# secondlaw-ai/skyrim

Hardware: AMD Instinct MI355X
Metric: 6-h forecast steps/sec on 721x1440 state, 1/2/4/8 MI355X; per-channel max rel-err vs ref (higher is better)
Workload: dtype f16; 1 GPU; Pangu 6-h autoregressive rollout, 721x1440x69 state (13 levels x 5 vars + 4 surface), random-init weights (64 M params), state resident in HBM, 1 ensemble membe; parallelism=single GPU, members=1, finite=True, rounding=compensated, term_plan=0x66f

## Files before the change

### skyrim_amd/csrc/attention.hip

```cpp
#include <cstdlib>
#include "gemm_dma.h"
#include "launchers.h"

namespace skp {

__device__ __forceinline__ int attn_key(int f, int row) {
    return f < 8 ? 32 * (f >> 1) + 8 * (row >> 2) + 4 * (f & 1) + (row & 3) : 128 + row;
}

__device__ __forceinline__ void attn_softmax_pv(f32x4 (&s)[9], const uint4 (&vf)[2][5], f32x4 (&o)[2], f32x4& osum) {
    typedef f16 T;
    const float LOG2E = 1.4426950408889634f;
    float mx = s[0][0];
#pragma unroll
    for (int f = 0; f < 9; ++f)
#pragma unroll
        for (int r = 0; r < 4; ++r) mx = fmaxf(mx, s[f][r]);
    mx = fmaxf(mx, __shfl_xor(mx, 16));
    mx = fmaxf(mx, __shfl_xor(mx, 32));
    const float mxl = mx * LOG2E;
#pragma unroll
    for (int f = 0; f < 9; ++f)
#pragma unroll
        for (int r = 0; r < 4; ++r) s[f][r] = __builtin_amdgcn_exp2f(__builtin_fmaf(s[f][r], LOG2E, -mxl));
    o[0] = f32x4{0.f, 0.f, 0.f, 0.f}; o[1] = f32x4{0.f, 0.f, 0.f, 0.f}; osum = f32x4{0.f, 0.f, 0.f, 0.f};
    const uint4 ones = make_uint4(0x3C003C00u, 0x3C003C00u, 0x3C003C00u, 0x3C003C00u);
#pragma unroll
    for (int kb = 0; kb < 5; ++kb) {
        float pv[8];
#pragma unroll
        for (int r = 0; r < 4; ++r) {
            pv[r] = s[2 * kb][r];
            pv[4 + r] = (kb < 4) ? s[(2 * kb + 1) % 9][r] : 0.f;
        }
        uint4 pf[1];
        split8<T, 1>(pv, pf);
#pragma unroll
        for (int df = 0; df < 2; ++df) o[df] = OpT<T>::mfma(as_v8<T>(vf[df][kb]), as_v8<T>(pf[0]), o[df]);
        osum = OpT<T>::mfma(as_v8<T>(ones), as_v8<T>(pf[0]), osum);
    }
}

constexpr int BT_ROW = 28, BT_COPY = 144 * BT_ROW + 120;

template <class TO, int NPL_O>
__global__ void __launch_bounds__(256) __attribute__((amdgpu_waves_per_eu(3, 3))) earth_attention2_kernel(const f16* __restrict__ q, const f16* __restrict__ k,
                                                              const f16* __restrict__ vt, const f16* __restrict__ bias_cmp, TO* __restrict__ out,
                                                              long long out_plane, int ld_out, int nW, int heads) {
    typedef f16 T;
    __shared__ __attribute__((aligned(16))) f16 tabs[4 * BT_COPY];
    const int lane = threadIdx.x & 63, wave = threadIdx.x >> 6;
    const int th = blockIdx.x;
    const int head = th % heads, type = th / heads;
    const int l15 = lane & 15, g = lane >> 4;
    {
        const f16* src = bias_cmp + (long long)th * 3456;
        for (int i = threadIdx.x; i < 3456; i += 256) {
            const int r = i / 24, e = i - 24 * r;
            const f16 v = src[i];
            if (e < 23) {
#pragma unroll
                for (int c = 0; c < 4; ++c) tabs[c * BT_COPY + r * BT_ROW + e + c] = v;
            }
        }
    }
    int koff[9];
#pragma unroll
    for (int f = 0; f < 9; ++f) {
        const int k0 = f < 8 ? 32 * (f >> 1) + 8 * g + 4 * (f & 1) : 128 + 4 * g;
        const int zk = k0 / 72, hk = (k0 / 12) % 6, wk0 = k0 % 12;
        koff[f] = 2 * ((2 * zk * 36 + 6 * hk) * BT_ROW + wk0);
    }
    __syncthreads();
    const char* tb = reinterpret_cast<const char*>(tabs);

    for (int wi = wave; wi < nW; wi += 4) {
        const int win = type * nW + wi;
        const long long base = (long long)win * heads + head;
        const T* qp = q + base * (WIN_TOKENS * HEAD_DIM) + l15 * HEAD_DIM + g * 8;
        const T* kp = k + base * (WIN_TOKENS * HEAD_DIM) + g * 8;
        const T* vp = vt + base * (WIN_TOKENS * HEAD_DIM) + (8 * (l15 >> 2) + (l15 & 3)) * WIN_TOKENS;

        uint4 kf[9];
#pragma unroll
        for (int f = 0; f < 9; ++f) kf[f] = *reinterpret_cast<const uint4*>(kp + attn_key(f, l15) * HEAD_DIM);
        uint4 vf[2][5];
#pragma unroll
        for (int df = 0; df < 2; ++df)
#pragma unroll
            for (int kb = 0; kb < 5; ++kb) {
                const T* s = vp + df * 4 * WIN_TOKENS;
                if (kb < 4) vf[df][kb] = *reinterpret_cast<const uint4*>(s + kb * 32 + g * 8);
                else { const uint2 lo = *reinterpret_cast<const uint2*>(s + 128 + g * 4); vf[df][kb] = make_uint4(lo.x, lo.y, 0, 0); }
            }
        uint4 qn = *reinterpret_cast<const uint4*>(qp);
#pragma unroll 1
        for (int qf = 0; qf < 9; ++qf) {
            const uint4 qv = qn;
            if (qf < 8) qn = *reinterpret_cast<const uint4*>(qp + (qf + 1) * 16 * HEAD_DIM);
            const int qi = 16 * qf + l15;
            const int zq = qi >= 72 ? 1 : 0, hq = (qi - 72 * zq) / 12, wq = qi - 72 * zq - 12 * hq;
            const int c = (wq + 1) & 3;
            const char* bq = tb + 2 * (c * BT_COPY + (zq * 36 + hq) * BT_ROW + (11 - wq) + c);
            uint2 bias[9];
#pragma unroll
            for (int f = 0; f < 9; ++f) bias[f] = *reinterpret_cast<const uint2*>(bq + koff[f]);

            f32x4 s[9];
#pragma unroll
            for (int f = 0; f < 9; ++f) {
                typedef f16 h4 __attribute__((ext_vector_type(4)));
                const h4 b = __builtin_bit_cast(h4, bias[f]);
                s[f] = OpT<T>::mfma(as_v8<T>(kf[f]), as_v8<T>(qv), f32x4{(float)b[0], (float)b[1], (float)b[2], (float)b[3]});
            }
            f32x4 o[2], osum;
            attn_softmax_pv(s, vf, o, osum);
            const float inv = __builtin_amdgcn_rcpf(osum[0]);
            TO* orow = out + blk_off((long long)win * WIN_TOKENS + qf * 16 + l15, head * HEAD_DIM, ld_out) + g * 8;
            const float y[8] = {o[0][0] * inv, o[0][1] * inv, o[0][2] * inv, o[0][3] * inv, o[1][0] * inv, o[1][1] * inv, o[1][2] * inv, o[1][3] * inv};
            store8_planes<TO, NPL_O>(orow, out_plane, y);
        }
    }
}


template <int C_, int PL_>
struct QaShape {
    static constexpr int C = C_, PL = PL_, KS = C / 32, NWAVES = 8, THREADS = 64 * NWAVES;
    static constexpr int BLK_KIB = KS * 2 * PL;
    static constexpr int W_BYTES = 3 * BLK_KIB * 1024;
    static constexpr int TAB_BYTES = (4 * BT_COPY * 2 + 1023) / 1024 * 1024;
    static constexpr int RING_BYTES = 6 * 1024;
    static constexpr int SMEM = W_BYTES + TAB_BYTES + 1024 + NWAVES * RING_BYTES;
    static_assert(SMEM <= 160 * 1024, "LDS");
};

struct QkvAttnArgs {
    const f16* xs;
    const int* widx;
    const f16* wf;
    const float* bias;
    const f16* bias_cmp;
    const f16* zrow;
    f16* out; long long out_plane;
    int nW, heads, types;
    float scale;
};

template <class S, int NPL_O>
__global__ void __launch_bounds__(S::THREADS) __attribute__((amdgpu_waves_per_eu(2, 2)))
qkv_attention_kernel(const QkvAttnArgs a) {
    typedef f16 T;
    constexpr int C = S::C, KS = S::KS, PL = S::PL;
    extern __shared__ __attribute__((aligned(16))) char smem[];
    char* wl = smem;
    f16* tabs = reinterpret_cast<f16*>(smem + S::W_BYTES);
    float* qb = reinterpret_cast<float*>(smem + S::W_BYTES + S::TAB_BYTES);
    const int tid = threadIdx.x, lane = tid & 63, l15 = lane & 15, g = lane >> 4;
    const int wave = __builtin_amdgcn_readfirstlane(tid >> 6);
    const int xcd = blockIdx.x & 7, slot = blockIdx.x >> 3;
    const int head = slot % a.heads, type = xcd + 8 * (slot / a.heads);
    if (type >= a.types) return;
    const int th = type * a.heads + head;
    {
        const unsigned lds_base = (unsigned)(size_t)smem;
#pragma unroll
        for (int which = 0; which < 3; ++which) {
            const f16* src = a.wf + ((long long)(which * a.heads + head) * S::BLK_KIB << 9) + lane * 8;
            for (int p = wave; p < S::BLK_KIB; p += S::NWAVES) glds16(src + (p << 9), lds_base + (unsigned)((which * S::BLK_KIB + p) << 10));
        }
        const f16* src = a.bias_cmp + (long long)th * 3456;
        constexpr int NT = (3456 + S::THREADS - 1) / S::THREADS;
        f16 tv[NT];
#pragma unroll
        for (int j = 0; j < NT; ++j) { const int i = tid + j * S::THREADS; tv[j] = src[i < 3456 ? i : 0]; }
#pragma unroll
        for (int j = 0; j < NT; ++j) {
            const int i = tid + j * S::THREADS;
            const int r = i / 24, e = i - 24 * r;
            if (i < 3456 && e < 23) {
#pragma unroll
                for (int c = 0; c < 4; ++c) tabs[c * BT_COPY + r * BT_ROW + e + c] = tv[j];
            }
        }
        if (tid < 96) qb[tid] = a.bias[(tid >> 5) * C + head * HEAD_DIM + (tid & 31)];
    }
    int koff[9];
#pragma unroll
    for (int f = 0; f < 9; ++f) {
        const int k0 = f < 8 ? 32 * (f >> 1) + 8 * g + 4 * (f & 1) : 128 + 4 * g;
        const int zk = k0 / 72, hk = (k0 / 12) % 6, wk0 = k0 % 12;
        koff[f] = 2 * ((2 * zk * 36 + 6 * hk) * BT_ROW + wk0);
    }
    int srcn[9];
    auto load_src = [&](int wi_) {
        const int w_ = type * a.nW + wi_;
#pragma unroll
        for (int f = 0; f < 9; ++f) srcn[f] = a.widx[w_ * WIN_TOKENS + attn_key(f, l15)];
    };
    load_src(wave < a.nW ? wave : 0);
    asm volatile("s_waitcnt vmcnt(0)" ::: "memory");
    __syncthreads();
    const char* tb = reinterpret_cast<const char*>(tabs);
    const char* wrd = wl + lane * 16;
    const unsigned ring_base = (unsigned)(size_t)smem + (unsigned)(S::W_BYTES + S::TAB_BYTES + 1024 + wave * S::RING_BYTES);
    const char* ring_rd = smem + S::W_BYTES + S::TAB_BYTES + 1024 + wave * S::RING_BYTES + lane * 16;

    for (int wi = wave; wi < a.nW; wi += S::NWAVES) {
        const int win = type * a.nW + wi;
        int src[9];
#pragma unroll
        for (int f = 0; f < 9; ++f) src[f] = srcn[f];
        typedef unsigned u32x9 __attribute__((ext_vector_type(9)));
        u32x9 qx, qy, qz, qw;
        uint4 kf[9];
        uint2 vh[9][2];
        const T* xp[3];
        int xstep[3];
        auto point = [&](int tg_) {
#pragma unroll
            for (int i = 0; i < 3; ++i) {
                const int r = src[3 * tg_ + i];
                xp[i] = r >= 0 ? a.xs + blk_off(r, g * 8, C) : a.zrow;
                xstep[i] = r >= 0 ? 512 : 0;
            }
        };
        auto fetch = [&](int ks) {
#pragma unroll
            for (int i = 0; i < 3; ++i) glds16(xp[i] + ks * xstep[i], ring_base + (unsigned)(((ks & 1) * 3 + i) << 10));
        };
        point(0);
        fetch(0);
        fetch(1);
#pragma unroll
        for (int tg = 0; tg < 3; ++tg) {
            f32x4 qa[3][2], ka[3][2], va[3][2];
#pragma unroll
            for (int i = 0; i < 3; ++i)
#pragma unroll
                for (int n = 0; n < 2; ++n) { qa[i][n] = f32x4{0.f, 0.f, 0.f, 0.f}; ka[i][n] = f32x4{0.f, 0.f, 0.f, 0.f}; va[i][n] = f32x4{0.f, 0.f, 0.f, 0.f}; }
#pragma unroll 1
            for (int ks = 0; ks < KS; ++ks) {
                if (ks + 1 < KS) asm volatile("s_waitcnt vmcnt(3)" ::: "memory");
                else asm volatile("s_waitcnt vmcnt(0)" ::: "memory");
                uint4 xf[3];
#pragma unroll
                for (int i = 0; i < 3; ++i) xf[i] = *reinterpret_cast<const uint4*>(ring_rd + (((ks & 1) * 3 + i) << 10));
                if (ks + 2 < KS) {
                    asm volatile("s_waitcnt lgkmcnt(0)" ::: "memory");
                    fetch(ks + 2);
                }
#pragma unroll
                for (int which = 0; which < 3; ++which)
#pragma unroll
                    for (int n = 0; n < 2; ++n)
#pragma unroll
                        for (int p = PL - 1; p >= 0; --p) {
                            const uint4 w = *reinterpret_cast<const uint4*>(wrd + ((((which * KS + ks) * 2 + n) * PL + p) << 10));
#pragma unroll
                            for (int i = 0; i < 3; ++i) {
                                if (which == 0) qa[i][n] = OpT<T>::mfma(as_v8<T>(w), as_v8<T>(xf[i]), qa[i][n]);
                                else if (which == 1) ka[i][n] = OpT<T>::mfma(as_v8<T>(w), as_v8<T>(xf[i]), ka[i][n]);
                                else va[i][n] = OpT<T>::mfma(as_v8<T>(xf[i]), as_v8<T>(w), va[i][n]);
                            }
                        }
            }
            if (tg < 2) {
                point(tg + 1);
                fetch(0);
                fetch(1);
            }
            float bq[8], bk[8], bv[2];
#pragma unroll
            for (int i = 0; i < 8; ++i) { bq[i] = qb[8 * g + i]; bk[i] = qb[32 + 8 * g + i]; }
#pragma unroll
            for (int df = 0; df < 2; ++df) bv[df] = qb[64 + 8 * (l15 >> 2) + 4 * df + (l15 & 3)];
#pragma unroll
            for (int i = 0; i < 3; ++i) {
                const int f = 3 * tg + i;
                float v[8];
                uint4 o[1];
#pragma unroll
                for (int r = 0; r < 4; ++r) { v[r] = (qa[i][0][r] + bq[r]) * a.scale; v[4 + r] = (qa[i][1][r] + bq[4 + r]) * a.scale; }
                split8<T, 1>(v, o);
                asm volatile("" : "+v"(o[0].x), "+v"(o[0].y), "+v"(o[0].z), "+v"(o[0].w));
                qx[f] = o[0].x; qy[f] = o[0].y; qz[f] = o[0].z; qw[f] = o[0].w;
#pragma unroll
                for (int r = 0; r < 4; ++r) { v[r] = ka[i][0][r] + bk[r]; v[4 + r] = ka[i][1][r] + bk[4 + r]; }
                split8<T, 1>(v, o);
                kf[f] = o[0];
#pragma unroll
                for (int df = 0; df < 2; ++df) {
                    const float u[4] = {va[i][df][0] + bv[df], va[i][df][1] + bv[df], va[i][df][2] + bv[df], va[i][df][3] + bv[df]};
                    uint2 h[1];
                    split4<T, 1>(u, h);
                    vh[f][df] = h[0];
                }
                asm volatile("" : "+v"(kf[f].x), "+v"(kf[f].y), "+v"(kf[f].z), "+v"(kf[f].w), "+v"(vh[f][0].x), "+v"(vh[f][0].y), "+v"(vh[f][1].x), "+v"(vh[f][1].y));
            }
        }
        uint4 vf[2][5];
#pragma unroll
        for (int df = 0; df < 2; ++df) {
#pragma unroll
            for (int kb = 0; kb < 4; ++kb) vf[df][kb] = make_uint4(vh[2 * kb][df].x, vh[2 * kb][df].y, vh[2 * kb + 1][df].x, vh[2 * kb + 1][df].y);
            vf[df][4] = make_uint4(vh[8][df].x, vh[8][df].y, 0, 0);
        }
        if (wi + S::NWAVES < a.nW) load_src(wi + S::NWAVES);
#pragma unroll 1
        for (int qf = 0; qf < 9; ++qf) {
            const uint4 qc = make_uint4(qx[qf], qy[qf], qz[qf], qw[qf]);
            const int qi = attn_key(qf, l15);
            const int zq = qi >= 72 ? 1 : 0, hq = (qi - 72 * zq) / 12, wq = qi - 72 * zq - 12 * hq;
            const int c = (wq + 1) & 3;
            const char* bqp = tb + 2 * (c * BT_COPY + (zq * 36 + hq) * BT_ROW + (11 - wq) + c);
            f32x4 s[9];
#pragma unroll
            for (int f = 0; f < 9; ++f) {
                typedef f16 h4 __attribute__((ext_vector_type(4)));
                const h4 b = __builtin_bit_cast(h4, *reinterpret_cast<const uint2*>(bqp + koff[f]));
                s[f] = OpT<T>::mfma(as_v8<T>(kf[f]), as_v8<T>(qc), f32x4{(float)b[0], (float)b[1], (float)b[2], (float)b[3]});
            }
            f32x4 o[2], osum;
            attn_softmax_pv(s, vf, o, osum);
            const float inv = __builtin_amdgcn_rcpf(osum[0]);
            T* orow = a.out + blk_off((long long)win * WIN_TOKENS + qi, head * HEAD_DIM, C) + g * 8;
            const float y[8] = {o[0][0] * inv, o[0][1] * inv, o[0][2] * inv, o[0][3] * inv, o[1][0] * inv, o[1][1] * inv, o[1][2] * inv, o[1][3] * inv};
            store8_planes<T, NPL_O>(orow, a.out_plane, y);
        }
    }
}

template <class S>
static hipError_t launch_qa(const QkvAttnArgs& a, int types, int out_planes, hipStream_t stream) {
    if (out_planes == 1) {
        auto kern = qkv_attention_kernel<S, 1>;
        hipError_t e = hipFuncSetAttribute(reinterpret_cast<const void*>(kern), hipFuncAttributeMaxDynamicSharedMemorySize, S::SMEM);
        if (e != hipSuccess) return e;
        hipLaunchKernelGGL(kern, dim3((unsigned)(8 * ((types + 7) / 8) * a.heads)), dim3(S::THREADS), S::SMEM, stream, a);
    } else {
        auto kern = qkv_attention_kernel<S, 2>;
        hipError_t e = hipFuncSetAttribute(reinterpret_cast<const void*>(kern), hipFuncAttributeMaxDynamicSharedMemorySize, S::SMEM);
        if (e != hipSuccess) return e;
        hipLaunchKernelGGL(kern, dim3((unsigned)(8 * ((types + 7) / 8) * a.heads)), dim3(S::THREADS), S::SMEM, stream, a);
    }
    return hipGetLastError();
}

hipError_t op_qkv_attention(const Geom& g, const BlockW<f16>& b, const int* widx, int res, const f16* Xs, const Work<PrecF16x3>& wk, hipStream_t s, int out_planes) {
    if (!b.bias_cmp || !(b.qkvh || b.qkvf)) return hipErrorInvalidValue;
    const int heads = res == 0 ? 6 : 12;
    QkvAttnArgs a{Xs, widx, b.qkvh ? b.qkvh : b.qkvf, b.qkv_b, b.bias_cmp, wk.zrow, wk.ao, wk.ao_plane, g.nW[res], heads, g.types[res], 0.17677669529663687f};
    if (b.qkvh) return res == 0 ? launch_qa<QaShape<192, 1>>(a, g.types[res], out_planes, s) : launch_qa<QaShape<384, 1>>(a, g.types[res], out_planes, s);
    if (res != 0) return hipErrorNotSupported;
    return launch_qa<QaShape<192, 2>>(a, g.types[res], out_planes, s);
}

template <class P>
hipError_t launch_attention(const AttnArgs<P>& a, hipStream_t stream) {
    constexpr int NPL_O = (P::NA > P::NW ? P::NA : P::NW);
    const int types = a.n_win / a.nW;
    if (a.out_planes == 1)
        hipLaunchKernelGGL((earth_attention2_kernel<typename P::T, 1>), dim3((unsigned)(types * a.heads)), dim3(256), 0, stream,
                           a.q, a.k, a.vt, a.bias_cmp, a.out, a.out_plane, a.ld_out, a.nW, a.heads);
    else
        hipLaunchKernelGGL((earth_attention2_kernel<typename P::T, NPL_O>), dim3((unsigned)(types * a.heads)), dim3(256), 0, stream,
                           a.q, a.k, a.vt, a.bias_cmp, a.out, a.out_plane, a.ld_out, a.nW, a.heads);
    return hipGetLastError();
}

template hipError_t launch_attention<PrecBF16x3>(const AttnArgs<PrecBF16x3>&, hipStream_t);
template hipError_t launch_attention<PrecF16x3>(const AttnArgs<PrecF16x3>&, hipStream_t);

}
```

### skyrim_amd/csrc/common.h

```cpp
#pragma once
#include <hip/hip_runtime.h>
#include <stdint.h>

namespace skp {

typedef _Float16 f16;
typedef __bf16 bf16;
typedef float f32x4 __attribute__((ext_vector_type(4)));
typedef f16 f16x8 __attribute__((ext_vector_type(8)));
typedef bf16 bf16x8 __attribute__((ext_vector_type(8)));

template <class T> struct OpT;
template <> struct OpT<f16> {
    typedef f16x8 v8;
    static __device__ __forceinline__ f32x4 mfma(v8 a, v8 b, f32x4 c) {
        return __builtin_amdgcn_mfma_f32_16x16x32_f16(a, b, c, 0, 0, 0);
    }
};
template <> struct OpT<bf16> {
    typedef bf16x8 v8;
    static __device__ __forceinline__ f32x4 mfma(v8 a, v8 b, f32x4 c) {
        return __builtin_amdgcn_mfma_f32_16x16x32_bf16(a, b, c, 0, 0, 0);
    }
};

template <class T>
__device__ __forceinline__ typename OpT<T>::v8 as_v8(const uint4& u) {
    return __builtin_bit_cast(typename OpT<T>::v8, u);
}

struct PrecBF16x3 { typedef bf16 T; static constexpr int NA = 2, NW = 2; };
struct PrecF16x3  { typedef f16 T;  static constexpr int NA = 2, NW = 2; };
struct PrecF16x2W { typedef f16 T;  static constexpr int NA = 1, NW = 2; };

__device__ __forceinline__ void load8(const float* p, float (&v)[8]) {
    const float4 a = *reinterpret_cast<const float4*>(p), b = *reinterpret_cast<const float4*>(p + 4);
    v[0] = a.x; v[1] = a.y; v[2] = a.z; v[3] = a.w; v[4] = b.x; v[5] = b.y; v[6] = b.z; v[7] = b.w;
}

template <class T, int NP>
__device__ __forceinline__ void split8(const float (&v)[8], uint4 (&out)[NP]) {
    typename OpT<T>::v8 h;
#pragma unroll
    for (int i = 0; i < 8; ++i) h[i] = (T)v[i];
    if constexpr (NP == 2) asm volatile("" : "+v"(h));
    out[0] = __builtin_bit_cast(uint4, h);
    if constexpr (NP == 2) {
        typename OpT<T>::v8 l;
#pragma unroll
        for (int i = 0; i < 8; ++i) l[i] = (T)(v[i] - (float)h[i]);
        out[1] = __builtin_bit_cast(uint4, l);
    }
}

template <class T, int NP>
__device__ __forceinline__ void split4(const float (&v)[4], uint2 (&out)[NP]) {
    typedef T t4 __attribute__((ext_vector_type(4)));
    t4 h;
#pragma unroll
    for (int i = 0; i < 4; ++i) h[i] = (T)v[i];
    if constexpr (NP == 2) asm volatile("" : "+v"(h));
    out[0] = __builtin_bit_cast(uint2, h);
    if constexpr (NP == 2) {
        t4 l;
#pragma unroll
        for (int i = 0; i < 4; ++i) l[i] = (T)(v[i] - (float)h[i]);
        out[1] = __builtin_bit_cast(uint2, l);
    }
}

template <class S>
__device__ __forceinline__ void store4(S* p, const float (&v)[4]) {
    if constexpr (sizeof(S) == 4) {
        *reinterpret_cast<float4*>(p) = make_float4(v[0], v[1], v[2], v[3]);
    } else {
        uint2 o[1];
        split4<S, 1>(v, o);
        *reinterpret_cast<uint2*>(p) = o[0];
    }
}

__device__ __host__ __forceinline__ long long blk_off(long long row, int col, int K) {
    return (((row >> 4) * (K >> 5) + (col >> 5)) << 9) + ((row & 15) << 5) + (col & 31);
}

template <class T, int NP>
__device__ __forceinline__ void store4_planes(T* p, long long plane, const float (&v)[4]) {
    uint2 o[NP];
    split4<T, NP>(v, o);
    *reinterpret_cast<uint2*>(p) = o[0];
    if constexpr (NP == 2) *reinterpret_cast<uint2*>(p + plane) = o[1];
}

template <class T, int NP>
__device__ __forceinline__ void store8_planes(T* p, long long plane, const float (&v)[8]) {
    uint4 o[NP];
    split8<T, NP>(v, o);
    *reinterpret_cast<uint4*>(p) = o[0];
    if constexpr (NP == 2) *reinterpret_cast<uint4*>(p + plane) = o[1];
}

__device__ __host__ __forceinline__ int perm8_col(int rho) {
    const int r = rho & 31;
    return (rho & ~31) + 8 * ((r >> 2) & 3) + 4 * (r >> 4) + (r & 3);
}

template <int BK>
__device__ __forceinline__ int lds_off(int row, int slot) {
    if constexpr (BK == 64) return row * 128 + ((slot ^ (row & 7)) << 4);
    else                    return row * 64 + ((slot ^ ((row >> 1) & 3)) << 4);
}

typedef float f32x2 __attribute__((ext_vector_type(2)));
__device__ __forceinline__ f32x2 gelu_erf2(f32x2 x) {
    f32x2 a;
    a.x = __builtin_amdgcn_fmed3f(__builtin_fabsf(x.x), 0.f, 5.9396970f);
    a.y = __builtin_amdgcn_fmed3f(__builtin_fabsf(x.y), 0.f, 5.9396970f);
    f32x2 p = __builtin_elementwise_fma(a, (f32x2)(-6.177511978e-07f), (f32x2)(1.091520153e-05f));
    p = __builtin_elementwise_fma(a, p, (f32x2)(-4.273382365e-05f));
    p = __builtin_elementwise_fma(a, p, (f32x2)(-4.982745158e-04f));
    p = __builtin_elementwise_fma(a, p, (f32x2)(7.545167115e-03f));
    p = __builtin_elementwise_fma(a, p, (f32x2)(-5.282834917e-02f));
    p = __builtin_elementwise_fma(a, p, (f32x2)(-4.591012597e-01f));
    p = __builtin_elementwise_fma(a, p, (f32x2)(-1.151117682e+00f));
    p = p * a;
    f32x2 t;
    t.x = 1.0f - __builtin_amdgcn_exp2f(p.x);
    t.y = 1.0f - __builtin_amdgcn_exp2f(p.y);
    t.x = __builtin_copysignf(t.x, x.x);
    t.y = __builtin_copysignf(t.y, x.y);
    return ((f32x2)(0.5f) * x) * ((f32x2)(1.0f) + t);
}
__device__ __forceinline__ float gelu_erf(float x) { return gelu_erf2((f32x2){x, x}).x; }
__device__ __forceinline__ f32x2 gelu_erf2e(f32x2 x) {
    f32x2 a;
    a.x = __builtin_amdgcn_fmed3f(__builtin_fabsf(x.x), 0.f, 5.9396970f);
    a.y = __builtin_amdgcn_fmed3f(__builtin_fabsf(x.y), 0.f, 5.9396970f);
    const f32x2 a2 = a * a;
    const f32x2 q01 = __builtin_elementwise_fma(a, (f32x2)(-4.591012597e-01f), (f32x2)(-1.151117682e+00f));
    const f32x2 q23 = __builtin_elementwise_fma(a, (f32x2)(7.545167115e-03f), (f32x2)(-5.282834917e-02f));
    const f32x2 q45 = __builtin_elementwise_fma(a, (f32x2)(-4.273382365e-05f), (f32x2)(-4.982745158e-04f));
    const f32x2 q67 = __builtin_elementwise_fma(a, (f32x2)(-6.177511978e-07f), (f32x2)(1.091520153e-05f));
    const f32x2 a4 = a2 * a2;
    const f32x2 q03 = __builtin_elementwise_fma(a2, q23, q01);
    const f32x2 q47 = __builtin_elementwise_fma(a2, q67, q45);
    f32x2 p = __builtin_elementwise_fma(a4, q47, q03);
    p = p * a;
    f32x2 t;
    t.x = 1.0f - __builtin_amdgcn_exp2f(p.x);
    t.y = 1.0f - __builtin_amdgcn_exp2f(p.y);
    t.x = __builtin_copysignf(t.x, x.x);
    t.y = __builtin_copysignf(t.y, x.y);
    return ((f32x2)(0.5f) * x) * ((f32x2)(1.0f) + t);
}
__device__ __forceinline__ void gelu_erf8(const f32x4& lo, const f32x4& hi, float (&v)[8]) {
    const f32x2 r0 = gelu_erf2((f32x2){lo[0], lo[1]}), r1 = gelu_erf2((f32x2){lo[2], lo[3]});
    const f32x2 r2 = gelu_erf2((f32x2){hi[0], hi[1]}), r3 = gelu_erf2((f32x2){hi[2], hi[3]});
    v[0] = r0.x; v[1] = r0.y; v[2] = r1.x; v[3] = r1.y; v[4] = r2.x; v[5] = r2.y; v[6] = r3.x; v[7] = r3.y;
}

constexpr int WIN_TOKENS = 144;
constexpr int HEAD_DIM = 32;

}
```

Before: 75.76 steps/s.

## Precompute attention lane geometry in LDS and prefetch next bias tile

The fused QKV-attention kernel now precomputes per-lane query geometry (bias-table offset and output offset) into a small LDS table instead of recomputing integer divisions per query fragment. It prefetches the next fragment's relative-position bias into registers while the current one runs softmax. The softmax row max uses permlane16/32 swap instructions with fmed3-based max in place of shuffles. The first K-step is peeled so accumulators are zero-initialised through the MFMA operand instead of explicit zeroing. The cost is more register pressure and a reshuffled LDS layout.

```diff
diff --git a/skyrim_amd/csrc/attention.hip b/skyrim_amd/csrc/attention.hip
--- a/skyrim_amd/csrc/attention.hip
+++ b/skyrim_amd/csrc/attention.hip
@@ -1,23 +1,27 @@
 #include <cstdlib>
+#include <type_traits>
 #include "gemm_dma.h"
 #include "launchers.h"
 
 namespace skp {
 
-__device__ __forceinline__ int attn_key(int f, int row) {
-    return f < 8 ? 32 * (f >> 1) + 8 * (row >> 2) + 4 * (f & 1) + (row & 3) : 128 + row;
-}
-
+template <bool SWAP>
 __device__ __forceinline__ void attn_softmax_pv(f32x4 (&s)[9], const uint4 (&vf)[2][5], f32x4 (&o)[2], f32x4& osum) {
     typedef f16 T;
     const float LOG2E = 1.4426950408889634f;
-    float mx = s[0][0];
+    float mx = SWAP ? max_raw(s[0][0], s[0][1]) : s[0][0];
 #pragma unroll
     for (int f = 0; f < 9; ++f)
 #pragma unroll
-        for (int r = 0; r < 4; ++r) mx = fmaxf(mx, s[f][r]);
-    mx = fmaxf(mx, __shfl_xor(mx, 16));
-    mx = fmaxf(mx, __shfl_xor(mx, 32));
+        for (int r = 0; r < 4; ++r)
+            if (!SWAP || 4 * f + r >= 2) mx = fmaxf(mx, s[f][r]);
+    if constexpr (SWAP) {
+        mx = xlane_max_swap<16>(mx);
+        mx = xlane_max_swap<32>(mx);
+    } else {
+        mx = fmaxf(mx, __shfl_xor(mx, 16));
+        mx = fmaxf(mx, __shfl_xor(mx, 32));
+    }
     const float mxl = mx * LOG2E;
 #pragma unroll
     for (int f = 0; f < 9; ++f)
@@ -41,7 +45,6 @@
     }
 }
 
-constexpr int BT_ROW = 28, BT_COPY = 144 * BT_ROW + 120;
 
 template <class TO, int NPL_O>
 __global__ void __launch_bounds__(256) __attribute__((amdgpu_waves_per_eu(3, 3))) earth_attention2_kernel(const f16* __restrict__ q, const f16* __restrict__ k,
@@ -114,7 +117,7 @@
                 s[f] = OpT<T>::mfma(as_v8<T>(kf[f]), as_v8<T>(qv), f32x4{(float)b[0], (float)b[1], (float)b[2], (float)b[3]});
             }
             f32x4 o[2], osum;
-            attn_softmax_pv(s, vf, o, osum);
+            attn_softmax_pv<false>(s, vf, o, osum);
             const float inv = __builtin_amdgcn_rcpf(osum[0]);
             TO* orow = out + blk_off((long long)win * WIN_TOKENS + qf * 16 + l15, head * HEAD_DIM, ld_out) + g * 8;
             const float y[8] = {o[0][0] * inv, o[0][1] * inv, o[0][2] * inv, o[0][3] * inv, o[1][0] * inv, o[1][1] * inv, o[1][2] * inv, o[1][3] * inv};
@@ -130,9 +133,11 @@
     static constexpr int BLK_KIB = KS * 2 * PL;
     static constexpr int W_BYTES = 3 * BLK_KIB * 1024;
     static constexpr int TAB_BYTES = (4 * BT_COPY * 2 + 1023) / 1024 * 1024;
+    static constexpr int GEO_BYTES = 9 * 64 * 8;
     static constexpr int RING_BYTES = 6 * 1024;
-    static constexpr int SMEM = W_BYTES + TAB_BYTES + 1024 + NWAVES * RING_BYTES;
-    static_assert(SMEM <= 160 * 1024, "LDS");
+    static constexpr int GEO_OFF = W_BYTES + TAB_BYTES, QB_OFF = GEO_OFF + GEO_BYTES, RING_OFF = GEO_OFF + 5 * 1024;
+    static constexpr int SMEM = RING_OFF + NWAVES * RING_BYTES;
+    static_assert(GEO_BYTES <= 4608 && GEO_OFF % 8 == 0 && QB_OFF + 96 * 4 <= RING_OFF && RING_OFF % 1024 == 0 && SMEM <= 160 * 1024, "LDS");
 };
 
 struct QkvAttnArgs {
@@ -155,7 +160,9 @@
     extern __shared__ __attribute__((aligned(16))) char smem[];
     char* wl = smem;
     f16* tabs = reinterpret_cast<f16*>(smem + S::W_BYTES);
-    float* qb = reinterpret_cast<float*>(smem + S::W_BYTES + S::TAB_BYTES);
+    float* qb = reinterpret_cast<float*>(smem + S::QB_OFF);
+    typedef unsigned u32x2 __attribute__((ext_vector_type(2)));
+    u32x2* geo = reinterpret_cast<u32x2*>(smem + S::GEO_OFF);
     const int tid = threadIdx.x, lane = tid & 63, l15 = lane & 15, g = lane >> 4;
     const int wave = __builtin_amdgcn_readfirstlane(tid >> 6);
     const int xcd = blockIdx.x & 7, slot = blockIdx.x >> 3;
@@ -184,6 +191,7 @@
             }
         }
         if (tid < 96) qb[tid] = a.bias[(tid >> 5) * C + head * HEAD_DIM + (tid & 31)];
+        for (int i = tid; i < 9 * 64; i += S::THREADS) { const uint2 e = attn_lane_geometry(i >> 6, i & 63, C); geo[i] = u32x2{e.x, e.y}; }
     }
     int koff[9];
 #pragma unroll
@@ -203,8 +211,13 @@
     __syncthreads();
     const char* tb = reinterpret_cast<const char*>(tabs);
     const char* wrd = wl + lane * 16;
-    const unsigned ring_base = (unsigned)(size_t)smem + (unsigned)(S::W_BYTES + S::TAB_BYTES + 1024 + wave * S::RING_BYTES);
-    const char* ring_rd = smem + S::W_BYTES + S::TAB_BYTES + 1024 + wave * S::RING_BYTES + lane * 16;
+    const unsigned ring_base = (unsigned)(size_t)smem + (unsigned)(S::RING_OFF + wave * S::RING_BYTES);
+    const char* ring_rd = smem + S::RING_OFF + wave * S::RING_BYTES + lane * 16;
+    const u32x2* geo_rd = geo + lane;
+    u32x2 g1 = geo_rd[0], g2 = geo_rd[64];
+    uint2 bn[9];
+#pragma unroll
+    for (int f = 0; f < 9; ++f) bn[f] = *reinterpret_cast<const uint2*>(tb + g1.x + koff[f]);
 
     for (int wi = wave; wi < a.nW; wi += S::NWAVES) {
         const int win = type * a.nW + wi;
@@ -235,12 +248,8 @@
 #pragma unroll
         for (int tg = 0; tg < 3; ++tg) {
             f32x4 qa[3][2], ka[3][2], va[3][2];
-#pragma unroll
-            for (int i = 0; i < 3; ++i)
-#pragma unroll
-                for (int n = 0; n < 2; ++n) { qa[i][n] = f32x4{0.f, 0.f, 0.f, 0.f}; ka[i][n] = f32x4{0.f, 0.f, 0.f, 0.f}; va[i][n] = f32x4{0.f, 0.f, 0.f, 0.f}; }
-#pragma unroll 1
-            for (int ks = 0; ks < KS; ++ks) {
+            auto kstep = [&](const int ks, auto first) {
+                constexpr bool FIRST = decltype(first)::value;
                 if (ks + 1 < KS) asm volatile("s_waitcnt vmcnt(3)" ::: "memory");
                 else asm volatile("s_waitcnt vmcnt(0)" ::: "memory");
                 uint4 xf[3];
@@ -250,6 +259,7 @@
                     asm volatile("s_waitcnt lgkmcnt(0)" ::: "memory");
                     fetch(ks + 2);
                 }
+                const f32x4 zero = {0.f, 0.f, 0.f, 0.f};
 #pragma unroll
                 for (int which = 0; which < 3; ++which)
 #pragma unroll
@@ -257,14 +267,19 @@
 #pragma unroll
                         for (int p = PL - 1; p >= 0; --p) {
                             const uint4 w = *reinterpret_cast<const uint4*>(wrd + ((((which * KS + ks) * 2 + n) * PL + p) << 10));
+                            const bool z = FIRST && p == PL - 1;
 #pragma unroll
                             for (int i = 0; i < 3; ++i) {
-                                if (which == 0) qa[i][n] = OpT<T>::mfma(as_v8<T>(w), as_v8<T>(xf[i]), qa[i][n]);
-                                else if (which == 1) ka[i][n] = OpT<T>::mfma(as_v8<T>(w), as_v8<T>(xf[i]), ka[i][n]);
-                                else va[i][n] = OpT<T>::mfma(as_v8<T>(xf[i]), as_v8<T>(w), va[i][n]);
+                                if (which == 0) qa[i][n] = OpT<T>::mfma(as_v8<T>(w), as_v8<T>(xf[i]), z ? zero : qa[i][n]);
+                                else if (which == 1) ka[i][n] = OpT<T>::mfma(as_v8<T>(w), as_v8<T>(xf[i]), z ? zero : ka[i][n]);
+                                else va[i][n] = OpT<T>::mfma(as_v8<T>(xf[i]), as_v8<T>(w), z ? zero : va[i][n]);
                             }
                         }
-            }
+            };
+            static_assert(KS > 2, "k-step 0 waits and fetches as every step but the last two does");
+            kstep(0, std::true_type{});
+#pragma unroll 1
+            for (int ks = 1; ks < KS; ++ks) kstep(ks, std::false_type{});
             if (tg < 2) {
                 point(tg + 1);
                 fetch(0);
@@ -307,24 +322,29 @@
             vf[df][4] = make_uint4(vh[8][df].x, vh[8][df].y, 0, 0);
         }
         if (wi + S::NWAVES < a.nW) load_src(wi + S::NWAVES);
+        char* owin = reinterpret_cast<char*>(a.out + (long long)win * (WIN_TOKENS * C) + head * (16 * HEAD_DIM));
 #pragma unroll 1
         for (int qf = 0; qf < 9; ++qf) {
             const uint4 qc = make_uint4(qx[qf], qy[qf], qz[qf], qw[qf]);
-            const int qi = attn_key(qf, l15);
-            const int zq = qi >= 72 ? 1 : 0, hq = (qi - 72 * zq) / 12, wq = qi - 72 * zq - 12 * hq;
-            const int c = (wq + 1) & 3;
-            const char* bqp = tb + 2 * (c * BT_COPY + (zq * 36 + hq) * BT_ROW + (11 - wq) + c);
+            const unsigned oy = g1.y;
             f32x4 s[9];
 #pragma unroll
             for (int f = 0; f < 9; ++f) {
                 typedef f16 h4 __attribute__((ext_vector_type(4)));
-                const h4 b = __builtin_bit_cast(h4, *reinterpret_cast<const uint2*>(bqp + koff[f]));
+                const h4 b = __builtin_bit_cast(h4, bn[f]);
                 s[f] = OpT<T>::mfma(as_v8<T>(kf[f]), as_v8<T>(qc), f32x4{(float)b[0], (float)b[1], (float)b[2], (float)b[3]});
             }
+            unsigned bx = g2.x;
+            asm volatile("" : "+v"(bx), "+v"(s[8][3]));
+#pragma unroll
+            for (int f = 0; f < 9; ++f) bn[f] = *reinterpret_cast<const uint2*>(tb + bx + koff[f]);
+            g1 = g2;
+            g2 = geo_rd[(qf < 7 ? qf + 2 : qf - 7) * 64];
+            __builtin_amdgcn_sched_barrier(0);
             f32x4 o[2], osum;
-            attn_softmax_pv(s, vf, o, osum);
+            attn_softmax_pv<true>(s, vf, o, osum);
             const float inv = __builtin_amdgcn_rcpf(osum[0]);
-            T* orow = a.out + blk_off((long long)win * WIN_TOKENS + qi, head * HEAD_DIM, C) + g * 8;
+            T* orow = reinterpret_cast<T*>(owin + oy);
             const float y[8] = {o[0][0] * inv, o[0][1] * inv, o[0][2] * inv, o[0][3] * inv, o[1][0] * inv, o[1][1] * inv, o[1][2] * inv, o[1][3] * inv};
             store8_planes<T, NPL_O>(orow, a.out_plane, y);
         }
diff --git a/skyrim_amd/csrc/common.h b/skyrim_amd/csrc/common.h
--- a/skyrim_amd/csrc/common.h
+++ b/skyrim_amd/csrc/common.h
@@ -27,6 +27,19 @@
 template <class T>
 __device__ __forceinline__ typename OpT<T>::v8 as_v8(const uint4& u) {
     return __builtin_bit_cast(typename OpT<T>::v8, u);
+}
+
+__device__ __forceinline__ float max_raw(float a, float b) {
+    float big = __builtin_inff();
+    asm("" : "+s"(big));
+    return __builtin_amdgcn_fmed3f(a, b, big);
+}
+template <int XOR>
+__device__ __forceinline__ float xlane_max_swap(float x) {
+    static_assert(XOR == 16 || XOR == 32, "one swap instruction per distance");
+    const unsigned u = __builtin_bit_cast(unsigned, x);
+    const auto r = XOR == 16 ? __builtin_amdgcn_permlane16_swap(u, u, false, false) : __builtin_amdgcn_permlane32_swap(u, u, false, false);
+    return max_raw(__builtin_bit_cast(float, (unsigned)r[0]), __builtin_bit_cast(float, (unsigned)r[1]));
 }
 
 struct PrecBF16x3 { typedef bf16 T; static constexpr int NA = 2, NW = 2; };
@@ -162,4 +175,16 @@
 constexpr int WIN_TOKENS = 144;
 constexpr int HEAD_DIM = 32;
 
+__device__ __host__ __forceinline__ int attn_key(int f, int row) {
+    return f < 8 ? 32 * (f >> 1) + 8 * (row >> 2) + 4 * (f & 1) + (row & 3) : 128 + row;
 }
+constexpr int BT_ROW = 28, BT_COPY = 144 * BT_ROW + 120;
+__device__ __host__ __forceinline__ uint2 attn_lane_geometry(int qf, int lane, int C) {
+    const int qi = attn_key(qf, lane & 15);
+    const int zq = qi >= 72 ? 1 : 0, hq = (qi - 72 * zq) / 12, wq = qi - 72 * zq - 12 * hq;
+    const int c = (wq + 1) & 3;
+    return make_uint2(2u * (unsigned)(c * BT_COPY + (zq * 36 + hq) * BT_ROW + (11 - wq) + c),
+                      2u * (unsigned)(blk_off(qi, 0, C) + (lane >> 4) * 8));
+}
+
+}
```

After: 73.74 steps/s. -2.7%, worse.
